# uzh-rpg/dagr

Hardware: AMD Instinct MI355X
Metric: events_per_sec (higher is better)
Workload: dtype f32; 1 GPU; dagr-s + --use_image --img_net resnet50, 640x480 synthetic S-uniform, B=8 windows/step x 100000 events (50 ms each), r=7, K=16, events->graph->GNN(+image fusion)->decoded head outputs->confidence mask + NMS (device); image_branch=in-line, engines=3

## Files before the change

dagr_amd/_lib.py:

```python
import ctypes
import os

_HERE = os.path.dirname(os.path.abspath(__file__))
LIB_PATH = os.path.join(_HERE, "lib", "libdagr_hip.so")

c_void_p = ctypes.c_void_p
c_i32 = ctypes.c_int32
c_i64 = ctypes.c_int64
c_size_t = ctypes.c_size_t
c_float = ctypes.c_float


class PoolDesc(ctypes.Structure):
    _fields_ = [("batch_size", c_i32), ("channels", c_i32), ("gx", c_i32), ("gy", c_i32), ("vx", c_float),
                ("vy", c_float), ("inv_w", c_float), ("inv_h", c_float), ("two_max", c_float), ("r00", c_float),
                ("r02", c_float), ("r11", c_float), ("r12", c_float), ("rx", c_i32), ("ry", c_i32), ("aggr", c_i32),
                ("append_pos", c_i32), ("keep_order", c_i32)]


class GraphDesc(ctypes.Structure):
    _fields_ = [("width", c_i32), ("height", c_i32), ("batch_size", c_i32), ("max_neighbors", c_i32),
                ("queue_size", c_i32), ("radius", c_i32), ("delta_t_us", c_i32), ("time_window", c_i32),
                ("max_events", c_i64)]

# ... 111 lines not shown
    "dagr_pool_argmax": (ctypes.c_int, [c_void_p, c_i32, c_void_p, c_i32, c_i32, c_void_p, c_i32, c_i32, c_void_p, c_void_p]),
    "dagr_pool_grad": (ctypes.c_int, [c_void_p, c_i32, c_i32, c_i32, c_void_p, c_void_p, c_void_p, c_i32, c_void_p, c_i32,
                                      c_void_p]),
    "dagr_to_dense_grad": (ctypes.c_int, [c_i32, c_i32, c_void_p, c_void_p, c_float, c_float, c_i32, c_i32, c_i32, c_void_p,
                                          c_void_p, c_i32, c_void_p]),
    "dagr_sample_features": (ctypes.c_int, [c_void_p, c_i32, c_void_p, c_void_p, c_i32, c_void_p, c_i32, c_i32, c_i32,
                                            c_i32, c_i32, c_i32, c_void_p, c_i32, c_i32, c_void_p]),
    "dagr_nms_batched": (ctypes.c_int, [c_void_p, c_void_p, c_void_p, c_void_p, c_i32, c_i32, c_float, c_float, c_void_p,
                                        c_void_p, c_void_p, c_void_p]),
    "dagr_heads_finish": (ctypes.c_int, [ctypes.POINTER(HeadScale), ctypes.POINTER(HeadScale), c_i32, c_i32, c_void_p,
                                         c_void_p, c_void_p]),
    "dagr_heads_finish_detect": (ctypes.c_int, [ctypes.POINTER(HeadScale), ctypes.POINTER(HeadScale), c_i32, c_i32, c_void_p,
                                                c_void_p, c_float, c_float, c_float, c_void_p, c_void_p, c_void_p]),
    "dagr_decode_heads": (ctypes.c_int, [c_void_p, c_i32, c_i32, c_float, c_void_p, c_i32, c_i32, c_float, c_i32, c_i32,
                                         c_void_p, c_void_p]),
    "dagr_postprocess": (ctypes.c_int, [c_void_p, c_i32, c_i32, c_i32, c_float, c_float, c_float, c_void_p, c_void_p,
                                        c_void_p]),
    "dagr_masked_lin": (ctypes.c_int, [c_void_p, c_void_p, c_void_p, c_void_p, c_void_p, c_i32, c_i64, c_i32, c_i32, c_void_p]),
    "dagr_masked_lin_no_bias": (ctypes.c_int, [c_void_p, c_void_p, c_void_p, c_void_p, c_i32, c_i64, c_i32, c_i32, c_void_p]),
    "dagr_masked_isdiff": (ctypes.c_int, [c_void_p, c_void_p, c_void_p, c_float, c_float, c_i64, c_i32, c_void_p]),
    "dagr_masked_inplace_BN": (ctypes.c_int, [c_void_p, c_void_p, c_void_p, c_void_p, c_void_p, c_void_p, c_void_p, c_float,
                                              c_i64, c_i32, c_void_p]),
    "dagr_downsample_events": (ctypes.c_int, [c_void_p, c_void_p, c_void_p, c_i32, c_void_p, c_i32, c_i32, c_void_p,
                                              c_void_p, c_void_p]),
    "dagr_spline_conv_l0_tiles_rows": (ctypes.c_int, [c_i32, c_i32, c_i32, c_i32, c_i32, c_i32, c_i32, c_i32, c_i32, c_float,
                                                      c_float, c_i64, c_i64, c_i32, c_void_p, c_void_p, c_void_p, c_void_p,
                                                      c_i32, c_void_p, c_i32, c_void_p, c_void_p, c_i32, c_void_p, c_i32,
                                                      c_void_p, c_void_p]),
    "dagr_async_graph_append": (ctypes.c_int, [ctypes.POINTER(GraphDesc), c_void_p, c_i64, c_i64, c_void_p, c_void_p,
                                               c_void_p, c_i64, c_void_p, c_i32, c_void_p, c_i32, c_i64, c_void_p, c_void_p,
                                               c_void_p, c_void_p, c_void_p, c_void_p, c_void_p, c_void_p, c_void_p, c_i32,
                                               c_i32, c_i32, c_void_p]),
    "dagr_async_update": (ctypes.c_int, [ctypes.POINTER(AsyncUpdateArgs), c_void_p]),
    "dagr_pool_l0_stream": (ctypes.c_int, [ctypes.POINTER(PoolDesc), c_void_p, c_i32, ctypes.POINTER(GraphDesc), c_void_p,
                                           c_void_p, c_void_p, c_void_p, c_i32, c_void_p, c_void_p, c_i64, c_i64, c_i64,
                                           c_void_p, c_void_p, c_void_p, c_void_p, c_i32, c_i32, c_void_p, c_void_p,
                                           c_void_p, c_void_p, c_void_p, c_void_p, c_void_p, c_i32, c_void_p]),
    "dagr_spline_conv_fused_lds_bytes": (c_size_t, [c_i32, c_i32]),
    "dagr_spline_conv_fused_passes": (c_i32, [c_i32, c_i32]),
    "dagr_spline_conv_fused": (ctypes.c_int, [c_void_p, c_i32, c_void_p, c_void_p, c_void_p, c_void_p, c_i32, c_i32,
                                              c_void_p, c_i32, c_i32, c_i32, c_i32, c_float, c_float, c_void_p,
                                              c_void_p, c_void_p, c_i32, c_i32, c_i32, c_void_p]),
    "dagr_spline_conv_fused_pool": (ctypes.c_int, [c_void_p, c_i32, c_void_p, c_void_p, c_void_p, c_void_p, c_i32, c_i32,
                                                   c_void_p, c_i32, c_i32, c_i32, c_i32, c_float, c_float, c_void_p,
                                                   c_void_p, c_void_p, c_i32, c_i32, c_i32, ctypes.POINTER(PoolDesc),
                                                   c_void_p, c_void_p, c_void_p, c_void_p, c_void_p]),
    "dagr_spline_conv_fused_multi": (ctypes.c_int, [c_void_p, c_i32, c_void_p]),
    "dagr_spline_conv_fused_pair": (ctypes.c_int, [c_void_p, c_i32, c_void_p, c_void_p, c_void_p, c_i32, c_i32, c_i32, c_i32,
                                                   c_float, c_float, c_i32, c_i32, c_void_p, c_void_p, c_void_p, c_void_p,
                                                   c_i32, c_void_p, c_void_p, c_void_p, c_void_p, c_i32, c_void_p]),
    "dagr_gemm_epilogue_workspace_bytes": (c_size_t, []),
    "dagr_gemm_epilogue": (ctypes.c_int, [c_void_p, c_i64, c_i32, c_i64, c_void_p, c_i32, c_void_p, c_void_p, c_i64, c_i32,
                                          c_void_p, c_i64, c_void_p, c_size_t, c_void_p]),
    "dagr_add_relu": (ctypes.c_int, [c_void_p, c_void_p, c_i64, c_void_p]),
    "dagr_bias_relu": (ctypes.c_int, [c_void_p, c_void_p, c_i64, c_i32, c_void_p]),
    "dagr_bias_silu": (ctypes.c_int, [c_void_p, c_void_p, c_i64, c_i32, c_void_p]),
    "dagr_bn_relu_maxpool": (ctypes.c_int, [c_void_p, c_i32, c_i32, c_i32, c_i32, c_void_p, c_void_p, c_void_p, c_void_p]),
    "dagr_gemm_bias_act": (ctypes.c_int, [c_void_p, c_i32, c_void_p, c_i32, c_void_p, c_i32, c_void_p, c_void_p,
                                          c_i32, c_i32, c_i32, c_i32, c_void_p]),
    "dagr_async_flops": (ctypes.c_int, [c_void_p, c_i32, c_void_p, c_void_p, c_void_p, c_void_p, c_void_p, c_i32, c_void_p,
                                        c_void_p]),
    "dagr_viz_workspace_bytes": (c_size_t, [c_i32, c_i32, c_i32]),
    "dagr_viz_render": (ctypes.c_int, [c_void_p, c_i32, c_i32, c_i32, c_void_p, c_i32, c_void_p, c_void_p, c_void_p,
                                       c_void_p, c_i32, c_void_p, c_void_p, c_void_p, c_i32, c_i32, c_void_p, c_i32,
                                       c_void_p, c_void_p, c_void_p, c_size_t, c_void_p]),
    "dagr_augment_workspace_bytes": (c_size_t, [c_i64]),
    "dagr_augment_events": (ctypes.c_int, [c_void_p, c_i32, c_i32, c_i32, c_void_p, c_i32, c_void_p, c_i32, c_void_p, c_i32,
                                           c_void_p, c_i64, c_void_p, c_void_p, c_void_p, c_void_p, c_void_p, c_void_p,
                                           c_void_p, c_size_t, c_void_p]),
    "dagr_augment_status": (ctypes.c_int, [c_void_p, c_void_p]),
    "dagr_augment_frames": (ctypes.c_int, [c_void_p, c_i32, c_i32, c_i32, c_i32, c_i32, c_i32, c_void_p, c_void_p,
                                           c_void_p]),
    "dagr_augment_boxes": (ctypes.c_int, [c_void_p, c_i32, c_i32, c_i32, c_void_p, c_void_p, c_i32, c_i32, c_void_p,
                                          c_void_p]),
}

_lib = None


def lib():
    global _lib
    if _lib is None:
        if not os.path.exists(LIB_PATH):
            raise RuntimeError(
                f"dagr_amd: {LIB_PATH} not found -- build it with `make` (or __graft_entry__.build()). "
                "There is no CPU fallback for the event-graph hot path.")
        handle = ctypes.CDLL(LIB_PATH)
        for name, (res, args) in SIGNATURES.items():
            fn = getattr(handle, name)
            fn.restype = res
            fn.argtypes = args
        _lib = handle
    return _lib


def check(rc, what=""):
    if rc != 0:
        msg = lib().dagr_last_error().decode("utf-8", "replace")
        raise RuntimeError(f"libdagr_hip {what} failed (status {rc}): {msg}")


def ptr(t):
    return None if t is None else c_void_p(t.data_ptr())


def cur_stream(device=None):
# ... 3 lines not shown
```

dagr_amd/csrc/gemm_lt.hip:

```cpp
#include <hipblaslt/hipblaslt.h>

#include <map>
#include <tuple>

#include "common.hpp"

namespace dagr {
namespace {

struct LtPlan {
    hipblasLtMatmulDesc_t desc = nullptr;
    hipblasLtMatrixLayout_t a = nullptr, b = nullptr, c = nullptr, d = nullptr;
    hipblasLtMatmulAlgo_t algo;
    size_t workspace = 0;
};

hipblasLtHandle_t lt_handle() {
    static hipblasLtHandle_t h = [] {
        hipblasLtHandle_t hh = nullptr;
        if (hipblasLtCreate(&hh) != HIPBLAS_STATUS_SUCCESS) hh = nullptr;
        return hh;
    }();
    return h;
}

}
}

using namespace dagr;

extern "C" size_t dagr_gemm_epilogue_workspace_bytes(void) { return (size_t)64 << 20; }

extern "C" int dagr_gemm_epilogue(const float *A, int64_t M, int32_t K, int64_t lda, const float *Wt, int32_t N,
                                  const float *bias, const float *R, int64_t ldr, int32_t act, float *D, int64_t ldd,
                                  void *workspace, size_t workspace_bytes, void *stream) {
    DAGR_CHECK_ARG(M >= 0 && K >= 1 && N >= 1 && lda >= K && ldd >= N && (!R || ldr >= N) && (act == 0 || act == 1), "bad sizes");
    if (M == 0) return DAGR_OK;
    DAGR_CHECK_ARG(A && Wt && D, "NULL pointer");
    hipblasLtHandle_t h = lt_handle();
    if (!h) { set_error("dagr_gemm_epilogue: hipblasLtCreate failed"); return DAGR_ERR_HIP; }
    using Key = std::tuple<int64_t, int, int, int64_t, int64_t, int64_t, int, int, int>;
    static thread_local std::map<Key, LtPlan> plans;
    const Key key{M, K, N, lda, R ? ldr : -1, ldd, act, bias ? 1 : 0, R ? 1 : 0};
    auto it = plans.find(key);
    if (it == plans.end()) {
        LtPlan p;
#define LT_OK(expr)                                                                                        \
    do {                                                                                                   \
        if ((expr) != HIPBLAS_STATUS_SUCCESS) { set_error("dagr_gemm_epilogue: " #expr " failed"); return DAGR_ERR_HIP; } \
    } while (0)
        LT_OK(hipblasLtMatmulDescCreate(&p.desc, HIPBLAS_COMPUTE_32F, HIP_R_32F));
        const hipblasOperation_t op_n = HIPBLAS_OP_N;
        LT_OK(hipblasLtMatmulDescSetAttribute(p.desc, HIPBLASLT_MATMUL_DESC_TRANSA, &op_n, sizeof(op_n)));
        LT_OK(hipblasLtMatmulDescSetAttribute(p.desc, HIPBLASLT_MATMUL_DESC_TRANSB, &op_n, sizeof(op_n)));
        hipblasLtEpilogue_t epi = act ? (bias ? HIPBLASLT_EPILOGUE_RELU_BIAS : HIPBLASLT_EPILOGUE_RELU)
                                      : (bias ? HIPBLASLT_EPILOGUE_BIAS : HIPBLASLT_EPILOGUE_DEFAULT);
        LT_OK(hipblasLtMatmulDescSetAttribute(p.desc, HIPBLASLT_MATMUL_DESC_EPILOGUE, &epi, sizeof(epi)));
        if (bias) {
            const hipDataType bt = HIP_R_32F;
            LT_OK(hipblasLtMatmulDescSetAttribute(p.desc, HIPBLASLT_MATMUL_DESC_BIAS_DATA_TYPE, &bt, sizeof(bt)));
            LT_OK(hipblasLtMatmulDescSetAttribute(p.desc, HIPBLASLT_MATMUL_DESC_BIAS_POINTER, &bias, sizeof(bias)));
        }
        LT_OK(hipblasLtMatrixLayoutCreate(&p.a, HIP_R_32F, (uint64_t)N, (uint64_t)K, (int64_t)N));
        LT_OK(hipblasLtMatrixLayoutCreate(&p.b, HIP_R_32F, (uint64_t)K, (uint64_t)M, lda));
        LT_OK(hipblasLtMatrixLayoutCreate(&p.c, HIP_R_32F, (uint64_t)N, (uint64_t)M, R ? ldr : ldd));
        LT_OK(hipblasLtMatrixLayoutCreate(&p.d, HIP_R_32F, (uint64_t)N, (uint64_t)M, ldd));
        hipblasLtMatmulPreference_t pref = nullptr;
        LT_OK(hipblasLtMatmulPreferenceCreate(&pref));
        const uint64_t max_ws = workspace ? (uint64_t)workspace_bytes : 0;
        LT_OK(hipblasLtMatmulPreferenceSetAttribute(pref, HIPBLASLT_MATMUL_PREF_MAX_WORKSPACE_BYTES, &max_ws, sizeof(max_ws)));
        constexpr int kCand = 16;
        hipblasLtMatmulHeuristicResult_t res[kCand];
        int found = 0;
        const hipblasStatus_t st = hipblasLtMatmulAlgoGetHeuristic(h, p.desc, p.a, p.b, p.c, p.d, pref, kCand, res, &found);
        hipblasLtMatmulPreferenceDestroy(pref);
        if (st != HIPBLAS_STATUS_SUCCESS || found < 1) {
            set_error("dagr_gemm_epilogue: the library offers no kernel for this GEMM + epilogue");
            return DAGR_ERR_UNSUPPORTED;
        }
        int best = 0;
        hipStreamCaptureStatus cap = hipStreamCaptureStatusNone;
        (void)hipStreamIsCapturing((hipStream_t)stream, &cap);
        if (found > 1 && cap == hipStreamCaptureStatusNone) {
            hipEvent_t e0, e1;
            if (hipEventCreate(&e0) == hipSuccess && hipEventCreate(&e1) == hipSuccess) {
                const float alpha = 1.0f, beta = R ? 1.0f : 0.0f;
                float best_ms = 0.f;
                for (int c = 0; c < found; c++) {
                    if (res[c].workspaceSize > workspace_bytes) continue;
                    bool ok = true;
                    float ms = 0.f;
                    for (int rep = 0; rep < 3 && ok; rep++) {
                        if (rep == 1) (void)hipEventRecord(e0, (hipStream_t)stream);
                        ok = hipblasLtMatmul(h, p.desc, &alpha, Wt, p.a, A, p.b, &beta, R ? (const void *)R : (const void *)D,
                                             p.c, D, p.d, &res[c].algo, workspace, workspace_bytes,
                                             (hipStream_t)stream) == HIPBLAS_STATUS_SUCCESS;
                    }
                    (void)hipEventRecord(e1, (hipStream_t)stream);
                    if (hipEventSynchronize(e1) != hipSuccess || !ok) continue;
                    (void)hipEventElapsedTime(&ms, e0, e1);
                    if (best_ms == 0.f || ms < best_ms) { best_ms = ms; best = c; }
                }
                (void)hipEventDestroy(e0);
                (void)hipEventDestroy(e1);
            }
        }
        p.algo = res[best].algo;
        p.workspace = res[best].workspaceSize;
        it = plans.emplace(key, p).first;
#undef LT_OK
    }
    LtPlan &p = it->second;
    if (bias && hipblasLtMatmulDescSetAttribute(p.desc, HIPBLASLT_MATMUL_DESC_BIAS_POINTER, &bias, sizeof(bias)) !=
                    HIPBLAS_STATUS_SUCCESS) {
        set_error("dagr_gemm_epilogue: setting the bias pointer failed");
        return DAGR_ERR_HIP;
    }
    DAGR_CHECK_ARG(p.workspace <= workspace_bytes, "workspace too small for the selected kernel");
    const float alpha = 1.0f, beta = R ? 1.0f : 0.0f;
    const hipblasStatus_t st = hipblasLtMatmul(h, p.desc, &alpha, Wt, p.a, A, p.b, &beta, R ? (const void *)R : (const void *)D,
                                               p.c, D, p.d, &p.algo, workspace, workspace_bytes, (hipStream_t)stream);
    if (st != HIPBLAS_STATUS_SUCCESS) {
        set_error("dagr_gemm_epilogue: hipblasLtMatmul failed");
        return DAGR_ERR_HIP;
    }
    return DAGR_OK;
}
```

dagr_amd/engine.py:

```python
import contextlib
import ctypes
import gc
import types

import numpy as np
import torch

from . import _lib
from .graph.ev_graph import WindowGraphBuilder

FUSED_PASSES_MAX_NODES = 1600


def _f32(v):
    return float(torch.as_tensor(v, dtype=torch.float32))


def _same_domain(a, b):
    return (a["rx"], a["ry"], a["den_x"], a["den_y"]) == (b["rx"], b["ry"], b["den_x"], b["den_y"]) \
        and torch.equal(a["remap"], b["remap"])


def _bn_affine(bn):
    m = bn.module
# ... 64 lines not shown
    rows = []
    for b in range(ty):
        for a in range(tx):
            rows.append(W[(win_x + a) + 5 * (win_y + b)][cols_in] * scale.view(1, -1))
    rows.append(conv.lin.weight.detach().float().t()[cols_in] * scale.view(1, -1))
    cskip = 0
    if skip is not None:
        lin, norm_skip = skip
        s_scale, s_shift = _bn_affine(norm_skip)
        ws = lin.mlp.weight.detach().float().t()
        if cols_skip is not None:
            ws = ws[list(cols_skip)]
        rows.append(ws * s_scale.view(1, -1))
        shift = shift + s_shift
        cskip = lin.mlp.in_features
    return cin, cskip, torch.cat(rows, 0).contiguous().to(device), shift.contiguous().to(device)


class _Conv1x1Gemm(torch.nn.Module):

    def __init__(self, conv, relu=False):
        super().__init__()
        cout, cin = conv.weight.shape[:2]
        self.stride = conv.stride[0]
        self.relu = relu
        self.register_buffer("wt", conv.weight.detach().reshape(cout, cin).t().contiguous())
        self.register_buffer("b", conv.bias.detach().clone() if conv.bias is not None else torch.zeros(cout, device=conv.weight.device))

    def forward(self, x, residual=None):
        if self.stride != 1:
            x = x[:, :, ::self.stride, ::self.stride]
        B, C, H, W = x.shape
        a = x.permute(0, 2, 3, 1).reshape(-1, C)
        N = self.wt.shape[1]
        r = None if residual is None else residual.permute(0, 2, 3, 1)
        if _LT["ok"] and a.is_cuda and a.dtype == torch.float32 and a.stride(1) == 1 \
                and (r is None or (r.is_contiguous() and tuple(r.shape) == (B, H, W, N))):
            y = torch.empty((a.shape[0], N), dtype=torch.float32, device=a.device)
            ws = _lt_workspace(a.device)
            act = 1 if (self.relu or r is not None) else 0
            rc = _lib.lib().dagr_gemm_epilogue(_lib.ptr(a), a.shape[0], C, a.stride(0), _lib.ptr(self.wt), N,
                                               _lib.ptr(self.b), _lib.ptr(r), N, act, _lib.ptr(y), N, _lib.ptr(ws),
                                               ws.numel(), _lib.cur_stream(a.device))
            if rc == 0:
                return y.view(B, H, W, -1).permute(0, 3, 1, 2)
            _LT["ok"] = False
        if residual is not None:
            y = torch.addmm(self.b, a, self.wt).view(B, H, W, -1).permute(0, 3, 1, 2)
            return _add_relu_(y, residual)
        y = torch._addmm_activation(self.b, a, self.wt) if self.relu else torch.addmm(self.b, a, self.wt)
        return y.view(B, H, W, -1).permute(0, 3, 1, 2)


_LT = {"ok": True, "ws": {}}


def _lt_workspace(device):
    key = str(device)
    if key not in _LT["ws"]:
        _LT["ws"][key] = torch.empty(int(_lib.lib().dagr_gemm_epilogue_workspace_bytes()), dtype=torch.uint8, device=device)
    return _LT["ws"][key]


def _gemmify_1x1(module):
    for name, child in list(module.named_children()):
        if isinstance(child, torch.nn.Conv2d) and child.kernel_size == (1, 1) and child.groups == 1 \
                and child.padding == (0, 0) and child.stride[0] == child.stride[1]:
            setattr(module, name, _Conv1x1Gemm(child))
        else:
            _gemmify_1x1(child)


def _add_relu_(y, z):
    if y.is_cuda and y.dtype == torch.float32 and z.dtype == torch.float32 and y.shape == z.shape \
            and y.stride() == z.stride() and y.data_ptr() % 16 == 0 and z.data_ptr() % 16 == 0 \
            and (y.is_contiguous() or y.is_contiguous(memory_format=torch.channels_last)):
        _lib.check(_lib.lib().dagr_add_relu(_lib.ptr(y), _lib.ptr(z), y.numel(), _lib.cur_stream(y.device)), "add_relu")
        return y
    return torch.relu_(y.add_(z))


def _bias_relu_(y, bias):
    C = y.shape[1]
    if y.is_cuda and y.dtype == torch.float32 and C % 4 == 0 and y.is_contiguous(memory_format=torch.channels_last) \
            and y.data_ptr() % 16 == 0 and bias.data_ptr() % 16 == 0:
        _lib.check(_lib.lib().dagr_bias_relu(_lib.ptr(y), _lib.ptr(bias), y.numel(), C, _lib.cur_stream(y.device)),
                   "bias_relu")
        return y
    return torch.relu_(y.add_(bias.view(1, -1, 1, 1)))


def _baseconv_forward(m, x):
    y = m.conv(x)
    b = m._bias
    C = y.shape[1]
    if y.is_cuda and y.dtype == torch.float32 and C % 4 == 0 and y.is_contiguous(memory_format=torch.channels_last) \
            and y.data_ptr() % 16 == 0 and b.data_ptr() % 16 == 0:
        _lib.check(_lib.lib().dagr_bias_silu(_lib.ptr(y), _lib.ptr(b), y.numel(), C, _lib.cur_stream(y.device)),
                   "bias_silu")
        return y
    return torch.nn.functional.silu(y.add_(b.view(1, -1, 1, 1)), inplace=True)


def _conv_bias_relu(blk, name, x):
    conv = getattr(blk, name)
    b = getattr(blk, "_" + name + "_bias", None)
    out = conv(x)
    if b is not None:
        return _bias_relu_(out, b)
    if getattr(conv, "relu", False):
        return out
    return blk.relu(out)


# ... 470 lines not shown
        return self.graph.node_count_ptr() if self._dev_mode else None

    def _sample(self, n_ptr, n_max, pos, batch, b64, fmap, out, coff):
        if self._feat_ready is not None:
            ready = self._feat_ready.get(id(fmap))
            if ready is None:
                raise RuntimeError("pipelined window: a sampled feature map has no ready-event (the image branch did not "
                                   "announce it) -- reading it would race with the image stream")
            torch.cuda.current_stream(self.device).wait_event(ready)
        Bf, C, h, w = fmap.shape
        nhwc = fmap.permute(0, 2, 3, 1)
        if not nhwc.is_contiguous():
            nhwc = nhwc.contiguous()
        self._keep.append(nhwc)
        _lib.check(self.L.dagr_sample_features(n_ptr, n_max, _lib.ptr(pos), _lib.ptr(batch), b64, _lib.ptr(nhwc), Bf, h,
                                               w, C, self.W, self.H, _lib.ptr(out), out.shape[1], coff,
                                               _lib.cur_stream(self.device)), "sample_features")

    def _fold_image_branch(self):
        import copy
        from torch.nn.utils.fusion import fuse_conv_bn_eval
        bb, head = self.model.backbone, self.model.head
        net = copy.deepcopy(bb.net).eval()
        cnn = copy.deepcopy(head.cnn_head).eval()

        def fold_block(blk):
            for ci, bi in (("conv1", "bn1"), ("conv2", "bn2"), ("conv3", "bn3")):
                if hasattr(blk, ci):
                    setattr(blk, ci, fuse_conv_bn_eval(getattr(blk, ci), getattr(blk, bi)))
                    setattr(blk, bi, torch.nn.Identity())
            if blk.downsample is not None:
                blk.downsample = torch.nn.Sequential(fuse_conv_bn_eval(blk.downsample[0], blk.downsample[1]))
        for name in ("layer1", "layer2", "layer3", "layer4"):
            for blk in getattr(net.module, name):
                fold_block(blk)
        for m in cnn.modules():
            if hasattr(m, "conv") and hasattr(m, "bn") and isinstance(m.bn, torch.nn.BatchNorm2d):
                m.conv = fuse_conv_bn_eval(m.conv, m.bn)
                m.bn = torch.nn.Identity()
                if isinstance(getattr(m, "act", None), torch.nn.SiLU) and m.conv.bias is not None:
                    m._bias = m.conv.bias.detach().clone().contiguous()
                    m.conv.bias = None
                    m.forward = types.MethodType(_baseconv_forward, m)
        net = net.to(memory_format=torch.channels_last)
        cnn = cnn.to(memory_format=torch.channels_last)
        for blkname in ("layer1", "layer2", "layer3", "layer4"):
            _gemmify_1x1(getattr(net.module, blkname))
            for blk in getattr(net.module, blkname):
                relu_convs = ("conv1", "conv2") if hasattr(blk, "conv3") else ("conv1",)
                for cname in relu_convs:
                    conv = getattr(blk, cname)
                    if isinstance(conv, _Conv1x1Gemm):
                        conv.relu = True
                    elif isinstance(conv, torch.nn.Conv2d) and conv.bias is not None:
                        setattr(blk, "_" + cname + "_bias", conv.bias.detach().clone().contiguous())
                        conv.bias = None
                blk.forward = types.MethodType(_bottleneck_forward if hasattr(blk, "conv3") else _basicblock_forward,
                                               blk)
        bn = net.module.bn1
        scale = (bn.weight.detach().float() / torch.sqrt(bn.running_var.detach().float() + bn.eps)).contiguous()
        shift = (bn.bias.detach().float() - bn.running_mean.detach().float() * scale).contiguous()
        net.module._stem_affine = (scale, shift)
        net.module.forward_features = types.MethodType(_resnet_features_forward, net.module)
        _gemmify_1x1(net.feature_dconv)
        _gemmify_1x1(net.output_dconv)
        self._net_f, self._cnn_f = net, cnn

    def _image_branch(self, image, on_feature=None):
        if self._net_f is None:
            self._fold_image_branch()
        bb, head = types.SimpleNamespace(net=self._net_f), types.SimpleNamespace(cnn_head=self._cnn_f)
        x = image.contiguous(memory_format=torch.channels_last)
        net = self._net_f
        if on_feature is not None:
            feats = [None] * len(net.feature_layers)

            def emit(name, t):
                if name in net.feature_layers:
                    j = net.feature_layers.index(name)
                    feats[j] = net.feature_dconv[j](t) if len(net.feature_dconv) > 0 else t
                    on_feature(j, feats[j])
            d = _resnet_features_forward(net.module, x, emit)
            outs = [d[l] for l in net.output_layers]
            if len(net.output_dconv) > 0:
                outs = [dconv(o) for o, dconv in zip(outs, net.output_dconv)]
        else:
            feats, outs = bb.net(x)
        outs = outs[-self.num_scales:]
        resized = [torch.nn.functional.interpolate(f, o) for f, o in zip(outs, self.out_sizes)]
        return feats, head.cnn_head(resized)

    def stage_image(self, image):
        self._keep = []
        self._img_feats, self._cnn_out = self._image_branch(image)

    def image_async(self, image, stream=None):
        cur = torch.cuda.current_stream(self.device)
        if stream is not None:
            self._img_stream = stream
        if self._img_stream is None:
            self._img_stream = torch.cuda.Stream(self.device)
        s = self._img_stream
        s.wait_stream(cur)
        with torch.cuda.stream(s):
            feats, cnn_out = self._image_branch(image)
            ev = torch.cuda.Event()
            ev.record(s)
        return feats, cnn_out, ev

# ... 545 lines not shown
```

include/dagr_hip.h:

```cpp
#ifndef DAGR_HIP_H
#define DAGR_HIP_H

#include <stddef.h>
#include <stdint.h>

#ifdef __cplusplus
extern "C" {
#endif

typedef enum {
    DAGR_OK = 0,
    DAGR_ERR_INVALID_ARG = -1,
    DAGR_ERR_HIP = -2,
    DAGR_ERR_WORKSPACE = -3,
    DAGR_ERR_UNSUPPORTED = -4
} dagr_status;

const char *dagr_last_error(void);
int dagr_version(void);
int dagr_device_count(void);

int dagr_format_events(const int16_t *xy , const int32_t *t , const int8_t *p ,
                       int64_t N, int32_t width, int32_t height, int32_t time_window,
                       float *pos_out , float *feat_out , void *stream);
// ... 220 lines not shown
                       float *grad_x, int32_t ldgx, void *stream);

int dagr_add_relu(float *y, const float *z, int64_t n, void *stream);
int dagr_bias_relu(float *y_nhwc, const float *bias, int64_t n, int32_t C, void *stream);
int dagr_bias_silu(float *y_nhwc, const float *bias, int64_t n, int32_t C, void *stream);
int dagr_bn_relu_maxpool(const float *x_nhwc, int32_t B, int32_t H, int32_t W, int32_t C, const float *scale,
                         const float *shift, float *y_nhwc, void *stream);

int dagr_sample_features(const int32_t *n_ptr, int32_t n_max, const float *pos, const void *batch,
                         int32_t batch_is_int64, const float *feat_nhwc, int32_t B, int32_t h, int32_t w, int32_t C,
                         int32_t width, int32_t height, float *out, int32_t ldo, int32_t coff, void *stream);

int dagr_nms_batched(const float *boxes, const float *scores, const int32_t *cls, const uint8_t *valid,
                     int32_t B, int32_t A, float iou_threshold, float class_offset,
                     int32_t *order_out, int32_t *keep_out, int32_t *n_keep, void *stream);

typedef struct dagr_head_scale {
    const int32_t *n_ptr; int32_t n_max;
    const float *pred; int32_t ld;
    const float *pos; const int32_t *batch;
    float vx, vy, stride; int32_t Hc, Wc;
    const float *cnn[3]; int32_t cnn_stride[3][4];
    float *dense;
} dagr_head_scale;
int dagr_heads_finish(const dagr_head_scale *scale0, const dagr_head_scale *scale1, int32_t batch_size, int32_t channels,
                      float *out, int32_t *status, void *stream);
int dagr_heads_finish_detect(const dagr_head_scale *scale0, const dagr_head_scale *scale1, int32_t batch_size,
                             int32_t channels, float *out, int32_t *status, float conf_threshold, float iou_threshold,
                             float class_offset, float *det, int32_t *n_keep, void *stream);
int dagr_decode_heads(const float *dense0, int32_t H0, int32_t W0, float stride0, const float *dense1, int32_t H1,
                      int32_t W1, float stride1, int32_t B, int32_t channels, float *out, void *stream);

int dagr_postprocess(const float *pred, int32_t B, int32_t A, int32_t num_classes, float conf_threshold,
                     float iou_threshold, float class_offset, float *det, int32_t *n_keep, void *stream);

int dagr_masked_lin(const int64_t *indices, const float *x_in, float *x_out, const float *weight, const float *bias,
                    int32_t add, int64_t K, int32_t Cin, int32_t Cout, void *stream);
int dagr_masked_lin_no_bias(const int64_t *indices, const float *x_in, float *x_out, const float *weight, int32_t add,
                            int64_t K, int32_t Cin, int32_t Cout, void *stream);
int dagr_masked_isdiff(int64_t *indices, const float *x_old, const float *x_new, float atol, float rtol, int64_t K,
                       int32_t C, void *stream);
int dagr_masked_inplace_BN(const int64_t *indices, const float *x, float *x_out, const float *running_mean,
                           const float *running_var, const float *weight, const float *bias, float eps, int64_t K,
                           int32_t C, void *stream);

int dagr_downsample_events(const int32_t *order, const int32_t *run_cell, const int32_t *run_end, int32_t n_runs,
                           const int8_t *polarity, int32_t fx, int32_t fy, float *change_map, uint8_t *keep,
                           void *stream);

size_t dagr_gemm_epilogue_workspace_bytes(void);
int dagr_gemm_epilogue(const float *A, int64_t M, int32_t K, int64_t lda, const float *Wt, int32_t N, const float *bias,
                       const float *R, int64_t ldr, int32_t act, float *D, int64_t ldd, void *workspace,
                       size_t workspace_bytes, void *stream);

enum { DAGR_FLOPS_ZERO = 0, DAGR_FLOPS_CONV = 1, DAGR_FLOPS_LINEAR = 2, DAGR_FLOPS_POOL = 3, DAGR_FLOPS_CARTESIAN = 4 };
typedef struct dagr_flops_module {
    int32_t kind, level, cin, cout, root, bias;
} dagr_flops_module;
int dagr_async_flops(const int32_t *deg, int32_t n_events, const int32_t *counts1, const int32_t *counts2,
                     const int32_t *counts3, const int32_t *counts4, const dagr_flops_module *mods, int32_t n_mods,
                     int64_t *out, void *stream);

size_t dagr_viz_workspace_bytes(int32_t F, int32_t H, int32_t W);
int dagr_viz_render(const uint8_t *images, int32_t n_images, int32_t H, int32_t W, const int32_t *frame_image, int32_t F,
                    const int32_t *ev_x, const int32_t *ev_y, const int8_t *ev_p, const int32_t *ev_ptr, int32_t n_events,
                    const double *alpha, const int32_t *boxes, const int32_t *box_ptr, int32_t n_boxes, int32_t linewidth,
                    const uint8_t *colors, int32_t n_colors, uint8_t *out, int32_t *status, void *workspace,
                    size_t workspace_bytes, void *stream);

typedef struct dagr_aug_params {
    int32_t flip, crop_on;
    int32_t crop_lo[2], crop_hi[2];
    float zoom;
    int32_t move[2];
} dagr_aug_params;
size_t dagr_augment_workspace_bytes(int64_t N);
int dagr_augment_events(const dagr_aug_params *params, int32_t B, int32_t W, int32_t H, const void *pos, int32_t pos_width,
                        const void *t, int32_t t_width, const void *p, int32_t p_width, const int32_t *sample_ptr, int64_t N,
                        int16_t *out_pos, void *out_t, void *out_p, int64_t *out_batch, int32_t *out_ptr,
                        int32_t *status, void *workspace, size_t workspace_bytes, void *stream);
int dagr_augment_status(const int32_t *status, void *stream);
int dagr_augment_frames(const dagr_aug_params *params, int32_t B, int32_t C, int32_t H, int32_t W, int32_t elem_bytes,
                        int32_t reference_crop, const void *in, void *out, void *stream);
int dagr_augment_boxes(const dagr_aug_params *params, int32_t B, int32_t W, int32_t H, const float *boxes,
                       const int64_t *box_batch, int32_t M, int32_t ld, float *out, void *stream);

int dagr_spiral_offsets(int32_t n, int32_t *dx_host, int32_t *dy_host);

#ifdef __cplusplus
}
#endif
#endif
```

Baseline: 146.3 million events/s.

## Replace ResNet 3x3 stride-1 convolutions with Winograd F(2x2,3x3) via batched hipBLASLt GEMM

Adds Winograd F(2x2,3x3) input and output transform kernels plus a strided-batched hipBLASLt GEMM entry point. The image backbone's eligible 3x3 convolutions (stride 1, pad 1, at least 128 in and out channels) are swapped for a path of input transform, 16 batched GEMMs and output transform, with bias and ReLU fused into the output step. The aim is to cut the multiply count of the fp32 image-branch convolutions. In exchange it allocates large 16xPxC intermediate buffers, adds extra memory traffic, and changes numerics slightly. It falls back to the original convolution if no GEMM kernel is available.

```diff
diff --git a/dagr_amd/_lib.py b/dagr_amd/_lib.py
--- a/dagr_amd/_lib.py
+++ b/dagr_amd/_lib.py
@@ -187,6 +187,11 @@
     "dagr_gemm_epilogue_workspace_bytes": (c_size_t, []),
     "dagr_gemm_epilogue": (ctypes.c_int, [c_void_p, c_i64, c_i32, c_i64, c_void_p, c_i32, c_void_p, c_void_p, c_i64, c_i32,
                                           c_void_p, c_i64, c_void_p, c_size_t, c_void_p]),
+    "dagr_gemm_batched": (ctypes.c_int, [c_void_p, c_i64, c_i32, c_i64, c_i64, c_void_p, c_i32, c_i64, c_void_p, c_i64, c_i64,
+                                         c_i32, c_void_p, c_size_t, c_void_p]),
+    "dagr_winograd_input_f2x3": (ctypes.c_int, [c_void_p, c_i32, c_i32, c_i32, c_i32, c_void_p, c_void_p]),
+    "dagr_winograd_output_f2x3": (ctypes.c_int, [c_void_p, c_i32, c_i32, c_i32, c_i32, c_void_p, c_i32, c_void_p,
+                                                 c_void_p]),
     "dagr_add_relu": (ctypes.c_int, [c_void_p, c_void_p, c_i64, c_void_p]),
     "dagr_bias_relu": (ctypes.c_int, [c_void_p, c_void_p, c_i64, c_i32, c_void_p]),
     "dagr_bias_silu": (ctypes.c_int, [c_void_p, c_void_p, c_i64, c_i32, c_void_p]),
diff --git a/dagr_amd/csrc/gemm_lt.hip b/dagr_amd/csrc/gemm_lt.hip
--- a/dagr_amd/csrc/gemm_lt.hip
+++ b/dagr_amd/csrc/gemm_lt.hip
@@ -24,30 +24,20 @@
     return h;
 }
 
-}
-}
-
-using namespace dagr;
-
-extern "C" size_t dagr_gemm_epilogue_workspace_bytes(void) { return (size_t)64 << 20; }
-
-extern "C" int dagr_gemm_epilogue(const float *A, int64_t M, int32_t K, int64_t lda, const float *Wt, int32_t N,
-                                  const float *bias, const float *R, int64_t ldr, int32_t act, float *D, int64_t ldd,
-                                  void *workspace, size_t workspace_bytes, void *stream) {
-    DAGR_CHECK_ARG(M >= 0 && K >= 1 && N >= 1 && lda >= K && ldd >= N && (!R || ldr >= N) && (act == 0 || act == 1), "bad sizes");
-    if (M == 0) return DAGR_OK;
-    DAGR_CHECK_ARG(A && Wt && D, "NULL pointer");
+int gemm_lt(const char *who, const float *A, int64_t M, int32_t K, int64_t lda, int64_t strideA, const float *Wt, int32_t N,
+            int64_t strideW, const float *bias, const float *R, int64_t ldr, int32_t act, float *D, int64_t ldd,
+            int64_t strideD, int32_t batch, void *workspace, size_t workspace_bytes, void *stream) {
     hipblasLtHandle_t h = lt_handle();
-    if (!h) { set_error("dagr_gemm_epilogue: hipblasLtCreate failed"); return DAGR_ERR_HIP; }
-    using Key = std::tuple<int64_t, int, int, int64_t, int64_t, int64_t, int, int, int>;
+    if (!h) { set_error(std::string(who) + ": hipblasLtCreate failed"); return DAGR_ERR_HIP; }
+    using Key = std::tuple<int64_t, int, int, int64_t, int64_t, int64_t, int, int, int, int, int64_t, int64_t, int64_t>;
     static thread_local std::map<Key, LtPlan> plans;
-    const Key key{M, K, N, lda, R ? ldr : -1, ldd, act, bias ? 1 : 0, R ? 1 : 0};
+    const Key key{M, K, N, lda, R ? ldr : -1, ldd, act, bias ? 1 : 0, R ? 1 : 0, batch, strideA, strideW, strideD};
     auto it = plans.find(key);
     if (it == plans.end()) {
         LtPlan p;
 #define LT_OK(expr)                                                                                        \
     do {                                                                                                   \
-        if ((expr) != HIPBLAS_STATUS_SUCCESS) { set_error("dagr_gemm_epilogue: " #expr " failed"); return DAGR_ERR_HIP; } \
+        if ((expr) != HIPBLAS_STATUS_SUCCESS) { set_error(std::string(who) + ": " #expr " failed"); return DAGR_ERR_HIP; } \
     } while (0)
         LT_OK(hipblasLtMatmulDescCreate(&p.desc, HIPBLAS_COMPUTE_32F, HIP_R_32F));
         const hipblasOperation_t op_n = HIPBLAS_OP_N;
@@ -65,6 +55,15 @@
         LT_OK(hipblasLtMatrixLayoutCreate(&p.b, HIP_R_32F, (uint64_t)K, (uint64_t)M, lda));
         LT_OK(hipblasLtMatrixLayoutCreate(&p.c, HIP_R_32F, (uint64_t)N, (uint64_t)M, R ? ldr : ldd));
         LT_OK(hipblasLtMatrixLayoutCreate(&p.d, HIP_R_32F, (uint64_t)N, (uint64_t)M, ldd));
+        if (batch > 1) {
+            const int64_t strides[4] = {strideW, strideA, strideD, strideD};
+            hipblasLtMatrixLayout_t layouts[4] = {p.a, p.b, p.c, p.d};
+            for (int l = 0; l < 4; l++) {
+                LT_OK(hipblasLtMatrixLayoutSetAttribute(layouts[l], HIPBLASLT_MATRIX_LAYOUT_BATCH_COUNT, &batch, sizeof(batch)));
+                LT_OK(hipblasLtMatrixLayoutSetAttribute(layouts[l], HIPBLASLT_MATRIX_LAYOUT_STRIDED_BATCH_OFFSET, &strides[l],
+                                                        sizeof(strides[l])));
+            }
+        }
         hipblasLtMatmulPreference_t pref = nullptr;
         LT_OK(hipblasLtMatmulPreferenceCreate(&pref));
         const uint64_t max_ws = workspace ? (uint64_t)workspace_bytes : 0;
@@ -75,7 +74,7 @@
         const hipblasStatus_t st = hipblasLtMatmulAlgoGetHeuristic(h, p.desc, p.a, p.b, p.c, p.d, pref, kCand, res, &found);
         hipblasLtMatmulPreferenceDestroy(pref);
         if (st != HIPBLAS_STATUS_SUCCESS || found < 1) {
-            set_error("dagr_gemm_epilogue: the library offers no kernel for this GEMM + epilogue");
+            set_error(std::string(who) + ": the library offers no kernel for this GEMM + epilogue");
             return DAGR_ERR_UNSUPPORTED;
         }
         int best = 0;
@@ -113,16 +112,48 @@
     LtPlan &p = it->second;
     if (bias && hipblasLtMatmulDescSetAttribute(p.desc, HIPBLASLT_MATMUL_DESC_BIAS_POINTER, &bias, sizeof(bias)) !=
                     HIPBLAS_STATUS_SUCCESS) {
-        set_error("dagr_gemm_epilogue: setting the bias pointer failed");
+        set_error(std::string(who) + ": setting the bias pointer failed");
         return DAGR_ERR_HIP;
     }
-    DAGR_CHECK_ARG(p.workspace <= workspace_bytes, "workspace too small for the selected kernel");
+    if (p.workspace > workspace_bytes) {
+        set_error(std::string(who) + ": workspace too small for the selected kernel");
+        return DAGR_ERR_INVALID_ARG;
+    }
     const float alpha = 1.0f, beta = R ? 1.0f : 0.0f;
     const hipblasStatus_t st = hipblasLtMatmul(h, p.desc, &alpha, Wt, p.a, A, p.b, &beta, R ? (const void *)R : (const void *)D,
                                                p.c, D, p.d, &p.algo, workspace, workspace_bytes, (hipStream_t)stream);
     if (st != HIPBLAS_STATUS_SUCCESS) {
-        set_error("dagr_gemm_epilogue: hipblasLtMatmul failed");
+        set_error(std::string(who) + ": hipblasLtMatmul failed");
         return DAGR_ERR_HIP;
     }
     return DAGR_OK;
 }
+
+}
+}
+
+using namespace dagr;
+
+extern "C" size_t dagr_gemm_epilogue_workspace_bytes(void) { return (size_t)64 << 20; }
+
+extern "C" int dagr_gemm_epilogue(const float *A, int64_t M, int32_t K, int64_t lda, const float *Wt, int32_t N,
+                                  const float *bias, const float *R, int64_t ldr, int32_t act, float *D, int64_t ldd,
+                                  void *workspace, size_t workspace_bytes, void *stream) {
+    DAGR_CHECK_ARG(M >= 0 && K >= 1 && N >= 1 && lda >= K && ldd >= N && (!R || ldr >= N) && (act == 0 || act == 1), "bad sizes");
+    if (M == 0) return DAGR_OK;
+    DAGR_CHECK_ARG(A && Wt && D, "NULL pointer");
+    return gemm_lt("dagr_gemm_epilogue", A, M, K, lda, 0, Wt, N, 0, bias, R, ldr, act, D, ldd, 0, 1, workspace,
+                   workspace_bytes, stream);
+}
+
+extern "C" int dagr_gemm_batched(const float *A, int64_t M, int32_t K, int64_t lda, int64_t strideA, const float *Wt,
+                                 int32_t N, int64_t strideW, float *D, int64_t ldd, int64_t strideD, int32_t batch,
+                                 void *workspace, size_t workspace_bytes, void *stream) {
+    DAGR_CHECK_ARG(M >= 0 && K >= 1 && N >= 1 && batch >= 0 && lda >= K && ldd >= N, "bad sizes");
+    DAGR_CHECK_ARG(batch <= 1 || (strideA >= (M - 1) * lda + K && strideW >= (int64_t)K * N && strideD >= (M - 1) * ldd + N) ||
+                       M == 0, "batch strides overlap the matrices");
+    if (M == 0 || batch == 0) return DAGR_OK;
+    DAGR_CHECK_ARG(A && Wt && D, "NULL pointer");
+    return gemm_lt("dagr_gemm_batched", A, M, K, lda, strideA, Wt, N, strideW, nullptr, nullptr, 0, 0, D, ldd, strideD, batch,
+                   workspace, workspace_bytes, stream);
+}
diff --git a/dagr_amd/csrc/winograd.hip b/dagr_amd/csrc/winograd.hip
--- /dev/null
+++ b/dagr_amd/csrc/winograd.hip
@@ -0,0 +1,166 @@
+#include "common.hpp"
+
+namespace dagr {
+namespace {
+
+template <int V>
+struct alignas(4 * V) Pack {
+    float v[V];
+};
+
+template <int V>
+__global__ __launch_bounds__(kBlock) void k_winograd_input_f2x3(const float *__restrict__ x, int H, int W, int C, int TH,
+                                                               int TW, int64_t P, float *__restrict__ Vt) {
+    const int CV = C / V;
+    const int64_t i = (int64_t)blockIdx.x * kBlock + threadIdx.x;
+    if (i >= P * CV) return;
+    const int cv = (int)(i % CV);
+    const int64_t p = i / CV;
+    const int tw = (int)(p % TW);
+    const int th = (int)((p / TW) % TH);
+    const int64_t b = p / ((int64_t)TW * TH);
+    const int y0 = 2 * th - 1, x0 = 2 * tw - 1;
+    Pack<V> d[4][4];
+#pragma unroll
+    for (int r = 0; r < 4; r++) {
+#pragma unroll
+        for (int s = 0; s < 4; s++) {
+            const int yy = y0 + r, xx = x0 + s;
+            if (yy >= 0 && yy < H && xx >= 0 && xx < W) {
+                d[r][s] = *reinterpret_cast<const Pack<V> *>(x + ((b * H + yy) * W + xx) * C + (int64_t)cv * V);
+            } else {
+#pragma unroll
+                for (int e = 0; e < V; e++) d[r][s].v[e] = 0.f;
+            }
+        }
+    }
+#pragma unroll
+    for (int s = 0; s < 4; s++) {
+#pragma unroll
+        for (int e = 0; e < V; e++) {
+            const float d0 = d[0][s].v[e], d1 = d[1][s].v[e], d2 = d[2][s].v[e], d3 = d[3][s].v[e];
+            d[0][s].v[e] = d0 - d2;
+            d[1][s].v[e] = d1 + d2;
+            d[2][s].v[e] = d2 - d1;
+            d[3][s].v[e] = d1 - d3;
+        }
+    }
+    const int64_t plane = P * C;
+    float *out = Vt + p * C + (int64_t)cv * V;
+#pragma unroll
+    for (int r = 0; r < 4; r++) {
+        Pack<V> o[4];
+#pragma unroll
+        for (int e = 0; e < V; e++) {
+            const float t0 = d[r][0].v[e], t1 = d[r][1].v[e], t2 = d[r][2].v[e], t3 = d[r][3].v[e];
+            o[0].v[e] = t0 - t2;
+            o[1].v[e] = t1 + t2;
+            o[2].v[e] = t2 - t1;
+            o[3].v[e] = t1 - t3;
+        }
+#pragma unroll
+        for (int s = 0; s < 4; s++) *reinterpret_cast<Pack<V> *>(out + (r * 4 + s) * plane) = o[s];
+    }
+}
+
+template <int V>
+__global__ __launch_bounds__(kBlock) void k_winograd_output_f2x3(const float *__restrict__ Mt, int H, int W, int K, int TH,
+                                                                int TW, int64_t P, const float *__restrict__ bias, int act,
+                                                                float *__restrict__ y) {
+    const int KV = K / V;
+    const int64_t i = (int64_t)blockIdx.x * kBlock + threadIdx.x;
+    if (i >= P * KV) return;
+    const int kv = (int)(i % KV);
+    const int64_t p = i / KV;
+    const int tw = (int)(p % TW);
+    const int th = (int)((p / TW) % TH);
+    const int64_t b = p / ((int64_t)TW * TH);
+    const int64_t plane = P * K;
+    const float *in = Mt + p * K + (int64_t)kv * V;
+    Pack<V> m[4][4];
+#pragma unroll
+    for (int r = 0; r < 4; r++) {
+#pragma unroll
+        for (int s = 0; s < 4; s++) m[r][s] = *reinterpret_cast<const Pack<V> *>(in + (r * 4 + s) * plane);
+    }
+    Pack<V> bv;
+#pragma unroll
+    for (int e = 0; e < V; e++) bv.v[e] = bias ? bias[kv * V + e] : 0.f;
+    Pack<V> o[2][2];
+#pragma unroll
+    for (int e = 0; e < V; e++) {
+        float s0[4], s1[4];
+#pragma unroll
+        for (int s = 0; s < 4; s++) {
+            s0[s] = m[0][s].v[e] + m[1][s].v[e] + m[2][s].v[e];
+            s1[s] = m[1][s].v[e] - m[2][s].v[e] - m[3][s].v[e];
+        }
+        float r00 = s0[0] + s0[1] + s0[2], r01 = s0[1] - s0[2] - s0[3];
+        float r10 = s1[0] + s1[1] + s1[2], r11 = s1[1] - s1[2] - s1[3];
+        r00 += bv.v[e]; r01 += bv.v[e]; r10 += bv.v[e]; r11 += bv.v[e];
+        if (act) {
+            r00 = r00 < 0.f ? 0.f : r00;
+            r01 = r01 < 0.f ? 0.f : r01;
+            r10 = r10 < 0.f ? 0.f : r10;
+            r11 = r11 < 0.f ? 0.f : r11;
+        }
+        o[0][0].v[e] = r00; o[0][1].v[e] = r01; o[1][0].v[e] = r10; o[1][1].v[e] = r11;
+    }
+#pragma unroll
+    for (int r = 0; r < 2; r++) {
+#pragma unroll
+        for (int s = 0; s < 2; s++) {
+            const int yy = 2 * th + r, xx = 2 * tw + s;
+            if (yy < H && xx < W)
+                *reinterpret_cast<Pack<V> *>(y + ((b * H + yy) * W + xx) * K + (int64_t)kv * V) = o[r][s];
+        }
+    }
+}
+
+inline bool aligned16(const void *p) { return ((uintptr_t)p % 16) == 0; }
+
+}
+}
+
+extern "C" int dagr_winograd_input_f2x3(const float *x_nhwc, int32_t B, int32_t H, int32_t W, int32_t C, float *V,
+                                        void *stream) {
+    using namespace dagr;
+    DAGR_CHECK_ARG(B >= 0 && H >= 1 && W >= 1 && C >= 1, "bad sizes");
+    if (B == 0) return DAGR_OK;
+    DAGR_CHECK_ARG(x_nhwc && V, "NULL pointer");
+    DAGR_CHECK_ARG(((uintptr_t)x_nhwc % 4) == 0 && ((uintptr_t)V % 4) == 0, "buffers must be 4-byte aligned");
+    const int TH = (H + 1) / 2, TW = (W + 1) / 2;
+    const int64_t P = (int64_t)B * TH * TW;
+    const bool vec = C % 4 == 0 && aligned16(x_nhwc) && aligned16(V);
+    const int64_t blocks = ceil_div(P * (vec ? C / 4 : C), (int64_t)kBlock);
+    DAGR_CHECK_ARG(blocks <= INT32_MAX, "map too large for one launch");
+    if (vec)
+        k_winograd_input_f2x3<4><<<(unsigned)blocks, kBlock, 0, (hipStream_t)stream>>>(x_nhwc, H, W, C, TH, TW, P, V);
+    else
+        k_winograd_input_f2x3<1><<<(unsigned)blocks, kBlock, 0, (hipStream_t)stream>>>(x_nhwc, H, W, C, TH, TW, P, V);
+    DAGR_CHECK_LAUNCH();
+    return DAGR_OK;
+}
+
+extern "C" int dagr_winograd_output_f2x3(const float *M, int32_t B, int32_t H, int32_t W, int32_t K, const float *bias,
+                                         int32_t act, float *y_nhwc, void *stream) {
+    using namespace dagr;
+    DAGR_CHECK_ARG(B >= 0 && H >= 1 && W >= 1 && K >= 1 && (act == 0 || act == 1), "bad sizes");
+    if (B == 0) return DAGR_OK;
+    DAGR_CHECK_ARG(M && y_nhwc, "NULL pointer");
+    DAGR_CHECK_ARG(((uintptr_t)M % 4) == 0 && ((uintptr_t)y_nhwc % 4) == 0 && ((uintptr_t)bias % 4) == 0,
+                   "buffers must be 4-byte aligned");
+    const int TH = (H + 1) / 2, TW = (W + 1) / 2;
+    const int64_t P = (int64_t)B * TH * TW;
+    const bool vec = K % 4 == 0 && aligned16(M) && aligned16(y_nhwc);
+    const int64_t blocks = ceil_div(P * (vec ? K / 4 : K), (int64_t)kBlock);
+    DAGR_CHECK_ARG(blocks <= INT32_MAX, "map too large for one launch");
+    if (vec)
+        k_winograd_output_f2x3<4><<<(unsigned)blocks, kBlock, 0, (hipStream_t)stream>>>(M, H, W, K, TH, TW, P, bias, act,
+                                                                                        y_nhwc);
+    else
+        k_winograd_output_f2x3<1><<<(unsigned)blocks, kBlock, 0, (hipStream_t)stream>>>(M, H, W, K, TH, TW, P, bias, act,
+                                                                                        y_nhwc);
+    DAGR_CHECK_LAUNCH();
+    return DAGR_OK;
+}
diff --git a/dagr_amd/engine.py b/dagr_amd/engine.py
--- a/dagr_amd/engine.py
+++ b/dagr_amd/engine.py
@@ -140,7 +140,53 @@
         return y.view(B, H, W, -1).permute(0, 3, 1, 2)
 
 
-_LT = {"ok": True, "ws": {}}
+def _winograd_pays(C, K, P=None):
+    return C >= 128 and K >= 128
+
+
+class _Conv3x3Winograd(torch.nn.Module):
+
+    def __init__(self, conv, relu=False):
+        super().__init__()
+        K, C = conv.weight.shape[:2]
+        self.relu = relu
+        g = conv.weight.detach().double()
+        G = torch.tensor([[1, 0, 0], [0.5, 0.5, 0.5], [0.5, -0.5, 0.5], [0, 0, 1]], dtype=torch.float64, device=g.device)
+        U = torch.einsum("ri,kcij,sj->rsck", G, g, G).reshape(16, C, K)
+        self.register_buffer("U", U.float().contiguous())
+        self.register_buffer("b", conv.bias.detach().float().clone().contiguous() if conv.bias is not None
+                             else torch.zeros(K, device=g.device))
+        self.conv = conv
+        if relu:
+            self.conv.bias = None
+
+    def forward(self, x):
+        B, C, H, W = x.shape
+        K = self.U.shape[2]
+        if _LT["wino_ok"] and x.is_cuda and x.dtype == torch.float32 and x.permute(0, 2, 3, 1).is_contiguous() \
+                and _winograd_pays(C, K, B * ((H + 1) // 2) * ((W + 1) // 2)):
+            L = _lib.lib()
+            P = B * ((H + 1) // 2) * ((W + 1) // 2)
+            st = _lib.cur_stream(x.device)
+            V = torch.empty((16, P, C), dtype=torch.float32, device=x.device)
+            M = torch.empty((16, P, K), dtype=torch.float32, device=x.device)
+            _lib.check(L.dagr_winograd_input_f2x3(_lib.ptr(x), B, H, W, C, _lib.ptr(V), st), "winograd_input_f2x3")
+            ws = _lt_workspace(x.device)
+            rc = L.dagr_gemm_batched(_lib.ptr(V), P, C, C, P * C, _lib.ptr(self.U), K, C * K, _lib.ptr(M), K, P * K, 16,
+                                     _lib.ptr(ws), ws.numel(), st)
+            if rc == 0:
+                y = torch.empty((B, K, H, W), dtype=torch.float32, device=x.device, memory_format=torch.channels_last)
+                _lib.check(L.dagr_winograd_output_f2x3(_lib.ptr(M), B, H, W, K, _lib.ptr(self.b), 1 if self.relu else 0,
+                                                       _lib.ptr(y), st), "winograd_output_f2x3")
+                return y
+            if rc != -4:
+                _lib.check(rc, "gemm_batched")
+            _LT["wino_ok"] = False
+        y = self.conv(x)
+        return _bias_relu_(y, self.b) if self.relu else y
+
+
+_LT = {"ok": True, "wino_ok": True, "ws": {}}
 
 
 def _lt_workspace(device):
@@ -148,6 +194,12 @@
     if key not in _LT["ws"]:
         _LT["ws"][key] = torch.empty(int(_lib.lib().dagr_gemm_epilogue_workspace_bytes()), dtype=torch.uint8, device=device)
     return _LT["ws"][key]
+
+
+def _winograd_eligible(conv):
+    return isinstance(conv, torch.nn.Conv2d) and conv.kernel_size == (3, 3) and conv.stride == (1, 1) \
+        and conv.padding == (1, 1) and conv.dilation == (1, 1) and conv.groups == 1 and conv.padding_mode == "zeros" \
+        and _winograd_pays(conv.in_channels, conv.out_channels)
 
 
 def _gemmify_1x1(module):
@@ -724,9 +776,13 @@
                     conv = getattr(blk, cname)
                     if isinstance(conv, _Conv1x1Gemm):
                         conv.relu = True
+                    elif _winograd_eligible(conv):
+                        setattr(blk, cname, _Conv3x3Winograd(conv, relu=True))
                     elif isinstance(conv, torch.nn.Conv2d) and conv.bias is not None:
                         setattr(blk, "_" + cname + "_bias", conv.bias.detach().clone().contiguous())
                         conv.bias = None
+                if not hasattr(blk, "conv3") and _winograd_eligible(blk.conv2):
+                    blk.conv2 = _Conv3x3Winograd(blk.conv2)
                 blk.forward = types.MethodType(_bottleneck_forward if hasattr(blk, "conv3") else _basicblock_forward,
                                                blk)
         bn = net.module.bn1
diff --git a/include/dagr_hip.h b/include/dagr_hip.h
--- a/include/dagr_hip.h
+++ b/include/dagr_hip.h
@@ -296,6 +296,13 @@
 int dagr_gemm_epilogue(const float *A, int64_t M, int32_t K, int64_t lda, const float *Wt, int32_t N, const float *bias,
                        const float *R, int64_t ldr, int32_t act, float *D, int64_t ldd, void *workspace,
                        size_t workspace_bytes, void *stream);
+int dagr_gemm_batched(const float *A, int64_t M, int32_t K, int64_t lda, int64_t strideA, const float *Wt, int32_t N,
+                      int64_t strideW, float *D, int64_t ldd, int64_t strideD, int32_t batch, void *workspace,
+                      size_t workspace_bytes, void *stream);
+
+int dagr_winograd_input_f2x3(const float *x_nhwc, int32_t B, int32_t H, int32_t W, int32_t C, float *V, void *stream);
+int dagr_winograd_output_f2x3(const float *M, int32_t B, int32_t H, int32_t W, int32_t K, const float *bias, int32_t act,
+                              float *y_nhwc, void *stream);
 
 enum { DAGR_FLOPS_ZERO = 0, DAGR_FLOPS_CONV = 1, DAGR_FLOPS_LINEAR = 2, DAGR_FLOPS_POOL = 3, DAGR_FLOPS_CARTESIAN = 4 };
 typedef struct dagr_flops_module {
```

New measurement: 148.7 million events/s, median of 3. About the same (+1.6%).
